# scylladb/seastar

Measured on AMD Instinct MI355X. Metric: GiB/s device-resident Internet checksum, 1500B-packet batches, 1/2/4/8 GPUs, higher is better.
Workload: dtype u8

## Files before the change

seastar_amd/csrc/sccsum.hip:

```cpp

#include <hip/hip_runtime.h>
#include "engine_seal.h"

#include <atomic>
#include <cctype>
#include <chrono>
#include <cstring>
#include <new>
#include <cstdint>
#include <cstdio>
#include <mutex>
#include <vector>

#include "host_launch.h"
#include "sccsum.h"
#include "sccsum_diag.h"

namespace sccsum {
namespace {

constexpr int kWave = 64;
constexpr int kBlock = 256;
constexpr int kWavesPerBlock = kBlock / kWave;
constexpr int kBlocksPerCU = 8;
// ... 800 lines not shown
        grp = group_of(wglob);
        const uint64_t rest = ntiles > nwaves ? ntiles - nwaves : 0;
        tiles_g = rest > grp ? static_cast<uint32_t>((rest - grp + kGroups - 1) / kGroups) : 0u;
        waves_g = static_cast<uint32_t>(nwaves / kGroups);
    }
    __device__ uint64_t end() const { return ntiles; }
    __device__ Ref ref(uint64_t tt) const {
        const bool sub = tt >= Q.tsplit;
        const uint64_t w = sub ? Q.tsplit + ((tt - Q.tsplit) >> Q.sub_log2) : tt;
        Ref r;
        r.q = 0;
        while (r.q + 1 < Q.nq && w >= Q.tile0[r.q + 1]) ++r.q;
        r.base = (w - Q.tile0[r.q]) * B;
        const uint64_t left = Q.n[r.q] - r.base;
        r.cnt = left < B ? static_cast<uint32_t>(left) : B;
        if (sub) {
            const uint32_t s0 = static_cast<uint32_t>((tt - Q.tsplit) & ((1u << Q.sub_log2) - 1u)) * Q.bsub;
            const uint32_t c = s0 < r.cnt ? r.cnt - s0 : 0u;
            r.base += s0 < r.cnt ? s0 : 0u;
            r.cnt = c < Q.bsub ? c : Q.bsub;
        }
        return r;
    }
    __device__ const uint8_t* bytes(const Ref& r) const { return Q.bytes[r.q]; }
    __device__ uint64_t bytes_len(const Ref& r) const { return Q.bytes_len[r.q]; }
    __device__ const uint64_t* off(const Ref& r) const { return Q.off[r.q]; }
    __device__ const uint32_t* len(const Ref& r) const { return Q.len[r.q]; }
    __device__ const uint32_t* seed(const Ref& r) const { return Q.seed[r.q]; }
    __device__ uint16_t* out(const Ref& r) const { return Q.out[r.q]; }
    __device__ uint8_t* status(const Ref& r) const { return Q.status[r.q]; }
    __device__ uint32_t tile_packets(const Ref&) const { return B; }
    __device__ bool is_store(const Ref&) const { return false; }
    __device__ uint32_t fill_flags(const Ref&, uint32_t flags) const { return flags; }
    __device__ uint32_t store_mode(const Ref&) const { return 0u; }

    struct Claim {
        uint32_t raw;
        uint64_t prev;
    };
    __device__ Claim claim_issue(uint64_t prev) {
        Claim c{0u, prev};
        if (heads != nullptr && lane == 0)
            c.raw = __hip_atomic_fetch_add(heads + grp * kHeadStride, 1u, __ATOMIC_RELAXED, __HIP_MEMORY_SCOPE_AGENT);
        return c;
    }
    __device__ uint64_t claim_resolve(const Claim& c) {
        if (heads == nullptr) return c.prev + nwaves;
        uint32_t d = c.raw;
        if (lane == 0 && d == tiles_g + waves_g - 1) {
            uint32_t* h = heads + grp * kHeadStride;
            __hip_atomic_store(h, 0u, __ATOMIC_RELAXED, __HIP_MEMORY_SCOPE_AGENT);
            asm volatile("s_waitcnt vmcnt(0)" ::: "memory");
            uint32_t* const groups_done = heads + kGroups * kHeadStride;
            const uint32_t gd = __hip_atomic_fetch_add(groups_done, 1u, __ATOMIC_RELAXED, __HIP_MEMORY_SCOPE_AGENT);
            if (gd == kGroups - 1) {
                __hip_atomic_store(groups_done, 0u, __ATOMIC_RELAXED, __HIP_MEMORY_SCOPE_AGENT);
                asm volatile("s_waitcnt vmcnt(0)" ::: "memory");
                __hip_atomic_store(done, ticket, __ATOMIC_RELAXED, __HIP_MEMORY_SCOPE_SYSTEM);
            }
        }
        d = __builtin_amdgcn_readfirstlane(d);
        return d < tiles_g ? nwaves + grp + static_cast<uint64_t>(kGroups) * d : ntiles;
    }
    __device__ uint64_t claim(uint64_t prev) { return claim_resolve(claim_issue(prev)); }
    __device__ uint64_t first() {
        uint64_t t = wglob;
        if (t >= ntiles && heads != nullptr) t = claim(t);
        return t;
    }
    __device__ bool ready(uint64_t) { return true; }
    __device__ bool wait_ready(uint64_t) { return true; }
    __device__ void retire(const Ref&) {}
};

constexpr uint32_t kEngineSlotWords = 64;
constexpr uint32_t kEngineCountSlots = 256;
constexpr uint32_t kEngineMaxRing = 1u << 16;
constexpr uint32_t kEngineDefaultRing = 1024;
#ifdef SCCSUM_AB_POLL_GROUP
constexpr uint32_t kPollGroup = SCCSUM_AB_POLL_GROUP;
#else
constexpr uint32_t kPollGroup = 16;
#endif
#ifdef SCCSUM_AB_NO_EXPECT
#define SCCSUM_HOT(x) (x)
#else
#define SCCSUM_HOT(x) __builtin_expect(!!(x), 1)
#endif
constexpr uint32_t kEdFirst = 0;
constexpr uint32_t kEdTiles = 1;
constexpr uint32_t kEdStep = 2;
constexpr uint32_t kEdNq = 3;
constexpr uint32_t kEdTile0 = 4;
constexpr uint32_t kEdQueue = 9;
constexpr uint32_t kEdKind = 41;
constexpr uint32_t kEdDep = 42;
constexpr uint32_t kEdIndex = 43;
constexpr uint32_t kStepSum = 0;
constexpr uint32_t kStepFillGen = 1;
constexpr uint32_t kStepFillStore = 2;
constexpr uint32_t kStoreTilePackets = 256;
constexpr uint32_t kEngineSyncEvery = 10;
#if defined(SCCSUM_AB_FILLSTORE_PLAIN) || defined(SCCSUM_AB_FILLSTORE_NORELEASE)
constexpr bool kStoreWT = false;
#else
constexpr bool kStoreWT = true;
#endif
constexpr uint32_t kEcPublished = 0, kEcStop = 8, kEcError = 16, kEcDone = 24;
constexpr uint64_t kErrIdle = 1, kErrDepWait = 2, kErrWalk = 3;
constexpr uint32_t kMpTiles = 0, kMpSteps = 8, kMpStop = 16, kMpToken = 24, kMpStamp = 32, kMirrorWords = 40;

struct EngineArgs {
    const uint64_t* hring;
    uint64_t* dring;
    uint64_t ring_mask;
    uint64_t* ctl;
    uint64_t* mirror;
    uint64_t* claims;
    uint32_t* counts;
    uint32_t* gdone;
    uint64_t* sdone;
    uint64_t idle_ticks;
    uint64_t dep_ticks;
};

__device__ __forceinline__ uint64_t rfl64(uint64_t x) {
    return static_cast<uint64_t>(static_cast<uint32_t>(__builtin_amdgcn_readfirstlane(static_cast<uint32_t>(x)))) |
           static_cast<uint64_t>(static_cast<uint32_t>(__builtin_amdgcn_readfirstlane(static_cast<uint32_t>(x >> 32))))
               << 32;
}
__device__ __forceinline__ uint64_t rl64(uint64_t x, uint32_t k) {
    return static_cast<uint64_t>(static_cast<uint32_t>(__builtin_amdgcn_readlane(static_cast<uint32_t>(x), k))) |
           static_cast<uint64_t>(static_cast<uint32_t>(__builtin_amdgcn_readlane(static_cast<uint32_t>(x >> 32), k)))
               << 32;
}

#ifdef SCCSUM_AB_NO_ENDPGM
__device__ __forceinline__ void engine_fault(uint64_t* ctl, uint32_t lane, uint64_t code) {
    if (lane == 0) __hip_atomic_store(ctl + kEcError, code, __ATOMIC_RELAXED, __HIP_MEMORY_SCOPE_SYSTEM);
}
#else
[[noreturn]] __device__ __forceinline__ void engine_fault(uint64_t* ctl, uint32_t lane, uint64_t code) {
    if (lane == 0) __hip_atomic_store(ctl + kEcError, code, __ATOMIC_RELAXED, __HIP_MEMORY_SCOPE_SYSTEM);
    asm volatile("s_waitcnt vmcnt(0)" ::: "memory");
    __builtin_amdgcn_endpgm();
}
#endif

struct WalkHit {
    uint64_t t, w;
};
__device__ __attribute__((noinline)) WalkHit engine_walk_far(const uint64_t* dring, uint64_t ring_mask,
                                                             const uint64_t* mirror, uint64_t* ctl, uint64_t below,
                                                             uint64_t v) {
    const uint32_t lane = __lane_id();
    uint64_t hs = 0;
    if (lane == 0) hs = __hip_atomic_load(mirror + kMpSteps, __ATOMIC_RELAXED, __HIP_MEMORY_SCOPE_AGENT);
    hs = rfl64(hs);
    uint64_t above = hs;
    bool bisect = false;
    uint64_t d = 1;
    for (;;) {
        uint64_t t;
        if (!bisect) {
            t = below + d;
            if (t >= above) {
                bisect = true;
                continue;
            }
        } else {
            if (above <= below + 1) break;
            t = below + (above - below) / 2;
        }
        uint64_t p = 0;
        if (lane == 0) p = __hip_atomic_load(dring + (t & ring_mask) * kEngineSlotWords + kEdStep, __ATOMIC_RELAXED,
                                             __HIP_MEMORY_SCOPE_AGENT);
        p = rfl64(p);
        if (seal_before(p, t, v)) {
            below = t;
            d <<= 1;
        } else {
            above = t;
            bisect = true;
        }
    }
    if (above >= hs) engine_fault(ctl, lane, kErrWalk);
    const uint64_t w = __hip_atomic_load(dring + (above & ring_mask) * kEngineSlotWords + lane, __ATOMIC_RELAXED,
                                         __HIP_MEMORY_SCOPE_AGENT);
    if (rl64(w, kEdIndex) != above || v < rl64(w, kEdFirst) || seal_before(rl64(w, kEdStep), above, v)) {
        engine_fault(ctl, lane, kErrWalk);
    }
    return WalkHit{above, w};
}

struct EngineSrc {
    static constexpr bool kEngine = true;
    const EngineArgs& E;
    const bool wt;
    uint32_t lane = 0, grp = 0;
    uint64_t pub = 0;
    uint64_t step = ~0ull, sfirst = 0, slast = 0;
    uint64_t dw = 0;
    uint64_t skind = 0, sdep = 0;
    uint64_t dep_seen = 0;
#ifdef SCCSUM_AB_TIMELINE
    unsigned long long ab[8] = {};
#endif
    struct Ref {
        uint32_t cnt, B, kind;
        uint64_t base, step, first, last;
        const uint8_t* bytes;
        uint64_t bytes_len;
        const uint64_t* off;
        const uint32_t* len;
        const uint32_t* seed;
        uint16_t* out;
        uint8_t* status;
    };
    __device__ EngineSrc(const EngineArgs& e, uint32_t flags) : E(e), wt((flags & kFlagEngineWT) != 0) {}
    __device__ void init(uint64_t wglob, uint64_t, uint32_t lane_) {
        lane = lane_;
        grp = group_of(wglob);
    }
    __device__ uint64_t end() const { return ~0ull; }
    struct Claim {
        uint64_t raw;
    };
    __device__ Claim claim_issue(uint64_t) {
        Claim c{0u};
        if (lane == 0) c.raw = __hip_atomic_fetch_add(E.claims + grp * (kHeadStride / 2), 1ull, __ATOMIC_RELAXED,
                                                      __HIP_MEMORY_SCOPE_AGENT);
        return c;
    }
    __device__ uint64_t claim_resolve(const Claim& c) {
        const uint64_t d = rfl64(c.raw);
        return grp + static_cast<uint64_t>(kGroups) * d;
    }
    __device__ uint64_t claim(uint64_t prev) { return claim_resolve(claim_issue(prev)); }
    __device__ uint64_t ctl_load(uint32_t w) {
        uint64_t v = 0;
        if (lane == 0) v = __hip_atomic_load(E.ctl + w, __ATOMIC_RELAXED, __HIP_MEMORY_SCOPE_SYSTEM);
        return rfl64(v);
    }
    __device__ uint64_t mload(uint32_t w) {
        uint64_t v = 0;
        if (lane == 0) v = __hip_atomic_load(E.mirror + w, __ATOMIC_RELAXED, __HIP_MEMORY_SCOPE_AGENT);
        return rfl64(v);
    }
    __device__ void poll() {
        uint32_t got = 0;
        if (lane == 0 && __hip_atomic_load(E.mirror + kMpToken, __ATOMIC_RELAXED, __HIP_MEMORY_SCOPE_AGENT) == 0) {
            uint64_t expect = 0;
            got = __hip_atomic_compare_exchange_strong(E.mirror + kMpToken, &expect, 1ull, __ATOMIC_RELAXED,
                                                       __ATOMIC_RELAXED, __HIP_MEMORY_SCOPE_AGENT)
                      ? 1u
                      : 0u;
        }
        if (!__builtin_amdgcn_readfirstlane(got)) return;
#ifdef SCCSUM_AB_TIMELINE
        ++ab[7];
#endif
        const uint64_t stop = ctl_load(kEcStop);
        const uint64_t hs = ctl_load(kEcPublished);
        uint64_t ms = mload(kMpSteps);
        const uint64_t ms0 = ms;
        uint64_t tiles = mload(kMpTiles);
        auto dslot = [&](uint64_t s) { return E.dring + (s & E.ring_mask) * kEngineSlotWords + lane; };
        auto put = [&](uint64_t s, uint64_t x) {
            __hip_atomic_store(dslot(s), x, __ATOMIC_RELAXED, __HIP_MEMORY_SCOPE_AGENT);
        };
        while (ms < hs) {
            const uint64_t g = hs - ms < kPollGroup ? hs - ms : kPollGroup;
            uint64_t w[kPollGroup];
#pragma unroll
            for (uint32_t k = 0; k < kPollGroup; ++k) {
                w[k] = k < g ? __hip_atomic_load(E.hring + ((ms + k) & E.ring_mask) * kEngineSlotWords + lane,
                                                 __ATOMIC_RELAXED, __HIP_MEMORY_SCOPE_SYSTEM)
                             : 0ull;
            }
#pragma unroll
            for (uint32_t k = 0; k < kPollGroup; ++k) {
                if (k < g) put(ms + k, w[k]);
            }
#pragma unroll
            for (uint32_t k = 0; k < kPollGroup; ++k) {
                if (k < g && static_cast<uint32_t>(rl64(w[k], kEdTiles)) == 0u && lane == 0) {
                    __hip_atomic_store(E.ctl + kEcDone + 8u * ((ms + k) & E.ring_mask), ms + k + 1, __ATOMIC_RELAXED,
                                       __HIP_MEMORY_SCOPE_SYSTEM);
                }
            }
#pragma unroll
            for (uint32_t k = 0; k < kPollGroup; ++k) {
                if (k + 1 == g) tiles = rl64(w[k], kEdFirst) + static_cast<uint32_t>(rl64(w[k], kEdTiles));
            }
            ms += g;
        }
        asm volatile("s_waitcnt vmcnt(0)" ::: "memory");
        if (lane == 0) __hip_atomic_store(E.mirror + kMpSteps, hs, __ATOMIC_RELAXED, __HIP_MEMORY_SCOPE_AGENT);
        asm volatile("s_waitcnt vmcnt(0)" ::: "memory");
        if (lane == 0) {
            __hip_atomic_store(E.mirror + kMpTiles, tiles, __ATOMIC_RELAXED, __HIP_MEMORY_SCOPE_AGENT);
            if (ms0 < hs) {
                __hip_atomic_store(E.mirror + kMpStamp, static_cast<uint64_t>(wall_clock64()), __ATOMIC_RELAXED,
                                   __HIP_MEMORY_SCOPE_AGENT);
            }
        }
        asm volatile("s_waitcnt vmcnt(0)" ::: "memory");
        if (lane == 0) {
            if (stop) __hip_atomic_store(E.mirror + kMpStop, 1ull, __ATOMIC_RELAXED, __HIP_MEMORY_SCOPE_AGENT);
            __hip_atomic_store(E.mirror + kMpToken, 0ull, __ATOMIC_RELAXED, __HIP_MEMORY_SCOPE_AGENT);
        }
    }
    __device__ bool published(uint64_t v) {
        if (SCCSUM_HOT(v < pub)) return true;
#ifdef SCCSUM_AB_TIMELINE
        ++ab[2];
#endif
        pub = mload(kMpTiles);
        return v < pub;
    }
    __device__ bool published_polled(uint64_t v) {
        if (published(v)) return true;
        poll();
        pub = mload(kMpTiles);
        return v < pub;
    }
    __device__ bool dep_ready(uint64_t v) {
        walk(v);
        if (SCCSUM_HOT(sdep == 0 || sdep <= dep_seen)) return true;
        const uint32_t slot = static_cast<uint32_t>((sdep - 1) % kEngineCountSlots);
        uint64_t d = 0;
        if (lane == 0) d = __hip_atomic_load(E.sdone + 8u * slot, __ATOMIC_RELAXED, __HIP_MEMORY_SCOPE_AGENT);
        d = rfl64(d);
        if (d < sdep) return false;
        dep_seen = sdep;
        return true;
    }
    __device__ bool ready(uint64_t v) { return published(v) && dep_ready(v); }
    __device__ bool wait_ready(uint64_t v) {
        if (ready(v)) return true;
        flush();
        const uint64_t t0 = static_cast<uint64_t>(wall_clock64());
#ifdef SCCSUM_AB_TIMELINE
        ++ab[0];
        struct Slept {
            unsigned long long* a;
            uint64_t t0;
            __device__ ~Slept() { a[1] += static_cast<uint64_t>(wall_clock64()) - t0; }
        } slept{ab, t0};
#endif
        for (;;) {
            const uint64_t stop = mload(kMpStop);
            const bool pubd = published_polled(v);
            if (pubd) {
                if (dep_ready(v)) return true;
                if (static_cast<uint64_t>(wall_clock64()) - t0 > E.dep_ticks) {
                    if (lane == 0) __hip_atomic_store(E.ctl + kEcError, kErrDepWait, __ATOMIC_RELAXED,
                                                      __HIP_MEMORY_SCOPE_SYSTEM);
                    return false;
                }
#ifdef SCCSUM_AB_DEP_SLEEP
                __builtin_amdgcn_s_sleep(SCCSUM_AB_DEP_SLEEP);
#else
                __builtin_amdgcn_s_sleep(32);
#endif
                continue;
            }
            if (stop) return false;
            const uint64_t now = static_cast<uint64_t>(wall_clock64());
            const uint64_t stamp = mload(kMpStamp);
            const uint64_t since = stamp > t0 ? stamp : t0;
            if (now > since && now - since > E.idle_ticks) {
                if (lane == 0) __hip_atomic_store(E.ctl + kEcError, kErrIdle, __ATOMIC_RELAXED,
                                                  __HIP_MEMORY_SCOPE_SYSTEM);
                return false;
            }
            __builtin_amdgcn_s_sleep(127);
        }
    }
    __device__ uint64_t first() {
        const uint64_t v = claim(0);
        return wait_ready(v) ? v : end();
    }
    __device__ void set_cursor(uint64_t t, uint64_t w) {
        step = t;
        dw = w;
        sfirst = rl64(w, kEdFirst);
        slast = sfirst + static_cast<uint32_t>(rl64(w, kEdTiles));
        skind = rl64(w, kEdKind);
        sdep = rl64(w, kEdDep);
    }
    __device__ bool walk(uint64_t v) {
        if (SCCSUM_HOT(step != ~0ull && v < slast)) return true;
#ifdef SCCSUM_AB_WALK_SEQ
        while (step == ~0ull || v >= slast) {
            const uint64_t t = step + 1;
            set_cursor(t, __hip_atomic_load(E.dring + (t & E.ring_mask) * kEngineSlotWords + lane, __ATOMIC_RELAXED,
                                            __HIP_MEMORY_SCOPE_AGENT));
        }
        return true;
#endif
#ifdef SCCSUM_AB_TIMELINE
        ++ab[3];
        const uint64_t w0 = static_cast<uint64_t>(wall_clock64());
        struct Walked {
            unsigned long long* a;
            uint64_t t0;
            __device__ ~Walked() { a[4] += static_cast<uint64_t>(wall_clock64()) - t0; }
        } walked{ab, w0};
#endif
        const uint64_t t = step + 1;
        const uint64_t w = __hip_atomic_load(E.dring + (t & E.ring_mask) * kEngineSlotWords + lane, __ATOMIC_RELAXED,
                                             __HIP_MEMORY_SCOPE_AGENT);
        if (SCCSUM_HOT(!seal_before(rl64(w, kEdStep), t, v) && rl64(w, kEdIndex) == t)) {
            set_cursor(t, w);
        } else {
            const WalkHit h = engine_walk_far(E.dring, E.ring_mask, E.mirror, E.ctl, t, v);
            set_cursor(rfl64(h.t), h.w);
        }
        return true;
    }
    __device__ Ref ref(uint64_t v) {
        Ref r;
        r.kind = static_cast<uint32_t>(skind);
        const uint64_t t_in = v - sfirst;
        const uint32_t nq = static_cast<uint32_t>(rl64(dw, kEdNq));
        uint32_t q = 0;
        while (q + 1 < nq && t_in >= rl64(dw, kEdTile0 + q + 1)) ++q;
        r.B = static_cast<uint32_t>(rl64(dw, kEdTiles) >> 32);
        r.base = (t_in - rl64(dw, kEdTile0 + q)) * r.B;
        const uint32_t qw = kEdQueue + 8u * q;
        const uint64_t left = rl64(dw, qw + 7) - r.base;
        r.cnt = left < r.B ? static_cast<uint32_t>(left) : r.B;
        r.bytes = reinterpret_cast<const uint8_t*>(rl64(dw, qw + 0));
        r.bytes_len = rl64(dw, qw + 1);
        r.off = reinterpret_cast<const uint64_t*>(rl64(dw, qw + 2));
        r.len = reinterpret_cast<const uint32_t*>(rl64(dw, qw + 3));
        r.seed = reinterpret_cast<const uint32_t*>(rl64(dw, qw + 4));
        r.out = reinterpret_cast<uint16_t*>(rl64(dw, qw + 5));
        r.status = reinterpret_cast<uint8_t*>(rl64(dw, qw + 6));
        r.step = step;
        r.first = sfirst;
        r.last = slast;
        return r;
    }
    __device__ const uint8_t* bytes(const Ref& r) const { return r.bytes; }
    __device__ uint64_t bytes_len(const Ref& r) const { return r.bytes_len; }
    __device__ const uint64_t* off(const Ref& r) const { return r.off; }
    __device__ const uint32_t* len(const Ref& r) const { return r.len; }
    __device__ const uint32_t* seed(const Ref& r) const { return r.seed; }
    __device__ uint16_t* out(const Ref& r) const { return r.out; }
    __device__ uint8_t* status(const Ref& r) const { return r.status; }
    __device__ uint32_t tile_packets(const Ref& r) const { return r.B; }
    __device__ bool is_store(const Ref& r) const { return (r.kind & 0xffu) == kStepFillStore; }
    __device__ uint32_t fill_flags(const Ref& r, uint32_t) const { return (r.kind >> 8) & 0xffu; }
    __device__ uint32_t store_mode(const Ref& r) const { return r.kind >> 16; }
    uint64_t pend_step = ~0ull, pend_first = 0, pend_last = 0;
    uint32_t pend = 0, pend_kind = 0;
#ifdef SCCSUM_AB_TIMELINE
    unsigned long long pend_t0 = 0, pend_t1 = 0;
#endif
    __device__ void flush() {
        if (pend == 0) return;
        const uint32_t k = pend;
        pend = 0;
#ifdef SCCSUM_AB_TIMELINE
        ++ab[5];
        struct Flushed {
            unsigned long long* a;
            uint64_t t0;
            __device__ ~Flushed() { a[6] += static_cast<uint64_t>(wall_clock64()) - t0; }
        } flushed{ab, static_cast<uint64_t>(wall_clock64())};
#endif
#ifdef SCCSUM_AB_TIMELINE
        if (lane == 0 && pend_step < kStepRec) {
            atomicMax(&g_step_grp[pend_step][grp], pend_t1);
            atomicMax(&g_step_xcd[pend_step][blockIdx.x & 7u][0], pend_t1);
            atomicMax(&g_step_xcd[pend_step][blockIdx.x & 7u][1], ~pend_t0);
        }
#endif
        if (lane != 0) return;
#ifdef SCCSUM_AB_FILLSTORE_NORELEASE
        if (false) {
#else
        if ((pend_kind & 0xffu) == kStepFillStore && !kStoreWT) {
#endif
            __builtin_amdgcn_fence(__ATOMIC_RELEASE, "");
        } else if (wt) {
            asm volatile("s_waitcnt vmcnt(0)" ::: "memory");
        } else {
            __builtin_amdgcn_fence(__ATOMIC_RELEASE, "agent");
        }
        const uint64_t fg = pend_first + ((grp + kGroups - pend_first % kGroups) % kGroups);
        const uint32_t expect = fg < pend_last ? static_cast<uint32_t>((pend_last - 1 - fg) / kGroups + 1) : 0u;
        const uint32_t slot = static_cast<uint32_t>(pend_step % kEngineCountSlots);
        uint32_t* const c = E.counts + (slot * kGroups + grp) * kHeadStride;
        const uint32_t x = __hip_atomic_fetch_add(c, k, __ATOMIC_RELAXED, __HIP_MEMORY_SCOPE_AGENT);
        if (x + k != expect) return;
        __hip_atomic_store(c, 0u, __ATOMIC_RELAXED, __HIP_MEMORY_SCOPE_AGENT);
        asm volatile("s_waitcnt vmcnt(0)" ::: "memory");
        uint32_t* const gd = E.gdone + slot * kHeadStride;
        const uint64_t ntl = pend_last - pend_first;
        const uint32_t groups = ntl < kGroups ? static_cast<uint32_t>(ntl) : kGroups;
        const uint32_t y = __hip_atomic_fetch_add(gd, 1u, __ATOMIC_RELAXED, __HIP_MEMORY_SCOPE_AGENT);
        if (y + 1 != groups) return;
        __hip_atomic_store(gd, 0u, __ATOMIC_RELAXED, __HIP_MEMORY_SCOPE_AGENT);
        __hip_atomic_store(E.sdone + 8u * slot, pend_step + 1, __ATOMIC_RELAXED, __HIP_MEMORY_SCOPE_AGENT);
        asm volatile("s_waitcnt vmcnt(0)" ::: "memory");
        __hip_atomic_store(E.ctl + kEcDone + 8u * (pend_step & E.ring_mask), pend_step + 1, __ATOMIC_RELAXED,
                           __HIP_MEMORY_SCOPE_SYSTEM);
    }
#ifdef SCCSUM_AB_TIMELINE
    __device__ void ab_stats(uint64_t wglob) {
        if (lane == 0 && wglob < kTimelineWaves)
            for (int i = 0; i < 8; ++i) g_engine_stats[wglob][i] = ab[i];
    }
#endif
    __device__ void retire(const Ref& r) {
        if (r.step != pend_step) {
            flush();
            pend_step = r.step;
            pend_first = r.first;
            pend_last = r.last;
            pend_kind = r.kind;
#ifdef SCCSUM_AB_TIMELINE
            pend_t0 = static_cast<uint64_t>(wall_clock64());
#endif
        }
        ++pend;
#ifdef SCCSUM_AB_TIMELINE
        pend_t1 = static_cast<uint64_t>(wall_clock64());
#endif
    }
};

template <bool kCoherent>
__device__ __forceinline__ uint32_t fill_ld32(const uint32_t* q) {
    if constexpr (kCoherent) {
        return __hip_atomic_load(gld(q), __ATOMIC_RELAXED, __HIP_MEMORY_SCOPE_AGENT);
    } else {
        return *gld(q);
    }
}
struct FillHead {
    uint32_t w, d0, d1, d2, d3;
};
template <bool kCoherent>
__device__ __forceinline__ FillHead fill_load(const uint8_t* p, const uint32_t* wp) {
    const uintptr_t a = reinterpret_cast<uintptr_t>(p);
    const uint32_t* d = reinterpret_cast<const uint32_t*>(a & ~uintptr_t(3));
    FillHead h;
    h.w = fill_ld32<kCoherent>(wp);
    h.d0 = fill_ld32<kCoherent>(d);
    h.d1 = fill_ld32<kCoherent>(d + 1);
    h.d2 = fill_ld32<kCoherent>(d + 2);
    h.d3 = fill_ld32<kCoherent>(d + 3);
    return h;
}
template <bool kCoherent, bool kWriteThrough = false>
__device__ __forceinline__ void fill_apply(uint8_t* p, uint32_t L, const FillHead& h, uint32_t mode) {
    const uint32_t sh = static_cast<uint32_t>(reinterpret_cast<uintptr_t>(p) & 3u);
    const uint32_t w = h.w, d0 = h.d0, d1 = h.d1, d2 = h.d2, d3 = h.d3;
    auto hbyte = [&](uint32_t k) {
        const uint32_t b = sh + k;
        const uint32_t dw = b < 4u ? d0 : (b < 8u ? d1 : (b < 12u ? d2 : d3));
        return (dw >> (8u * (b & 3u))) & 0xffu;
    };
    const uint32_t ihl = hbyte(0) & 0xfu;
    const uint32_t ip_len = (hbyte(2) << 8) | hbyte(3);
    const uint32_t fragw = (hbyte(6) << 8) | hbyte(7);
    const uint32_t proto = hbyte(9);
    const uint32_t l4_off = 4u * ihl;
    const uint32_t l4_end = ip_len < L ? ip_len : L;
    const bool atomic = !(L < ip_len || l4_off > l4_end || (fragw & 0x1fffu) * 8u + l4_end > 65535u ||
                          (fragw & 0x3fffu) != 0u || ihl < 5u);
    const uint32_t l4_len = l4_off > l4_end ? 0u : l4_end - l4_off;
    if (mode & SCCSUM_FILL_IP) store_field<kWriteThrough>(p + 10, w);
    if (!atomic) return;
    if (mode & SCCSUM_FILL_L4) {
        const uint32_t fo = proto == 17u ? 6u : (proto == 6u ? 16u : 0u);
        if (fo != 0u && l4_len >= fo + 2u) store_field<kWriteThrough>(p + l4_off + fo, w >> 16);
    }
    if ((mode & SCCSUM_FILL_ICMP_ECHO) && proto == 1u && l4_len >= 8u) {
        uint8_t* ih = p + l4_off;
        const uintptr_t ia = reinterpret_cast<uintptr_t>(ih);
        const uint32_t type = (fill_ld32<kCoherent>(reinterpret_cast<const uint32_t*>(ia & ~uintptr_t(3))) >>
                               (8u * static_cast<uint32_t>(ia & 3u))) & 0xffu;
        if (type == 8u) {
            store_field<kWriteThrough>(ih, 0u);
// ... 1505 lines not shown
    }
}

bool engine_all_done(sccsum_engine* e) {
    const uint64_t n = e->next_step.load(std::memory_order_relaxed);
    while (e->done_floor < n && engine_done(e, e->done_floor)) ++e->done_floor;
    return e->done_floor >= n;
}

int engine_check(const sccsum_engine* e, const sccsum_batch* batches, uint32_t nbatch, bool fill) {
    if (nbatch == 0 || nbatch > SCCSUM_ENGINE_MAX_BATCHES || !batches) return SCCSUM_EINVAL;
    for (uint32_t i = 0; i < nbatch; ++i) {
        const sccsum_batch& x = batches[i];
        if (e->frames && x.d_seed) return SCCSUM_EINVAL;
        if (!x.n) continue;
        const bool ok = e->frames
                            ? sccsum::batch_ok<true>(x.d_bytes, x.d_off, x.d_len, nullptr, x.d_out, x.d_status, 0)
                            : sccsum::batch_ok<false>(x.d_bytes, x.d_off, x.d_len, x.d_seed, x.d_out, x.d_status, 0);
        if (!ok) return SCCSUM_EINVAL;
        if (fill && !x.d_out) return SCCSUM_EINVAL;
    }
    return SCCSUM_OK;
}

bool engine_room(sccsum_engine* e, uint32_t k, uint64_t* need) {
    const uint64_t last = e->next_step.load(std::memory_order_relaxed) + k - 1;
    if (last < e->limit) return true;
    const uint64_t target = last - e->limit;
    while (e->done_floor <= target && engine_done(e, e->done_floor)) ++e->done_floor;
    if (e->done_floor > target) return true;
    *need = e->done_floor;
    return false;
}

uint64_t engine_tile(const sccsum_engine* e, const sccsum_batch* batches, uint32_t nbatch, uint32_t max_len) {
    uint64_t n_total = 0, bytes_total = 0;
    for (uint32_t i = 0; i < nbatch; ++i) {
        n_total += batches[i].n;
        bytes_total += batches[i].n ? batches[i].bytes_len : 0;
    }
    return sccsum::packets_per_tile(n_total, sccsum::packet_bytes(n_total, bytes_total, max_len), e->waves,
                                    sccsum::t_knobs);
}

uint64_t engine_put(sccsum_engine* e, const sccsum_batch* batches, uint32_t nbatch, uint64_t kind, uint64_t dep,
                    uint64_t B) {
    if ((kind & 0xffu) == sccsum::kStepFillStore) B = sccsum::kStoreTilePackets;
    const uint64_t s = e->next_step.load(std::memory_order_relaxed);
    uint64_t* const d = e->ring_h + (s & (e->ring - 1u)) * sccsum::kEngineSlotWords;
    uint64_t tile0[SCCSUM_ENGINE_MAX_BATCHES + 1] = {};
    uint32_t nq = 0;
    for (uint32_t i = 0; i < nbatch; ++i) {
        const sccsum_batch& x = batches[i];
        if (!x.n) continue;
        const uint32_t q = nq++;
        uint64_t* w = d + sccsum::kEdQueue + 8u * q;
        w[0] = reinterpret_cast<uint64_t>(x.d_bytes);
        w[1] = x.bytes_len;
        w[2] = reinterpret_cast<uint64_t>(x.d_off);
        w[3] = reinterpret_cast<uint64_t>(x.d_len);
        w[4] = e->frames ? 0u : reinterpret_cast<uint64_t>(x.d_seed);
        w[5] = reinterpret_cast<uint64_t>(x.d_out);
        w[6] = reinterpret_cast<uint64_t>(x.d_status);
        w[7] = x.n;
        tile0[q + 1] = tile0[q] + (x.n + B - 1) / B;
    }
    const uint64_t ntiles = tile0[nq];
    d[sccsum::kEdFirst] = e->next_first;
    d[sccsum::kEdTiles] = ntiles | (B << 32);
    d[sccsum::kEdStep] = sccsum::engine_seal(s, e->next_first + ntiles);
    d[sccsum::kEdIndex] = s;
    d[sccsum::kEdNq] = nq ? nq : 1;
    for (uint32_t q = 0; q <= SCCSUM_ENGINE_MAX_BATCHES; ++q) d[sccsum::kEdTile0 + q] = tile0[q];
    d[sccsum::kEdKind] = kind;
    d[sccsum::kEdDep] = dep;
    int sync = sccsum::t_knobs.engine_sync_every;
    if (sync < 0) sync = ntiles >= 2 * e->waves ? static_cast<int>(sccsum::kEngineSyncEvery) : 0;
    if (dep == 0 && sync > 0 && s > 0 && s % static_cast<uint64_t>(sync) == 0 && e->last_tiled != ~0ull) {
        d[sccsum::kEdDep] = e->last_tiled + 1;
    }
    if (ntiles) e->last_tiled = s;
    e->next_first += ntiles;
    e->next_step.store(s + 1, std::memory_order_release);
    __atomic_store_n(e->ctl_h + sccsum::kEcPublished, s + 1, __ATOMIC_SEQ_CST);
    return s;
}

template <class Put>
int engine_publish(sccsum_engine* e, uint32_t k, uint64_t timeout_ns, const Put& put) {
    const uint64_t t0 = now_ns();
    ProducerRecord* pr = nullptr;
    if (e->producer_limit) {
        uint64_t run;
        {
            std::lock_guard<std::mutex> g(e->mu);
            if (!e->running) return SCCSUM_EINVAL;
            run = e->run;
        }
        pr = &producer_record(e, run);
        while (pr->n >= e->producer_limit) {
            const uint64_t oldest = pr->steps[pr->head];
            const uint64_t spent = now_ns() - t0;
            const int rc = engine_wait_done(e, oldest, spent < timeout_ns ? timeout_ns - spent : 0);
            if (rc != SCCSUM_OK) return rc;
            pr->head = (pr->head + 1) % sccsum::kEngineCountSlots;
            --pr->n;
        }
    }
    for (;;) {
        uint64_t need = 0;
        {
            std::lock_guard<std::mutex> g(e->mu);
            if (!e->running) return SCCSUM_EINVAL;
            if (const int rc = engine_error(e)) return rc;
            if (engine_room(e, k, &need)) {
                put();
                if (pr) {
                    pr->steps[(pr->head + pr->n) % sccsum::kEngineCountSlots] =
                        e->next_step.load(std::memory_order_relaxed) - 1;
                    ++pr->n;
                }
                return SCCSUM_OK;
            }
        }
        const uint64_t spent = now_ns() - t0;
        const int rc = engine_wait_done(e, need, spent < timeout_ns ? timeout_ns - spent : 0);
        if (rc != SCCSUM_OK) return rc;
    }
}

int engine_ms(uint32_t ms, uint32_t dflt, uint64_t* ticks) {
    const uint64_t v = ms ? ms : dflt;
    if (v > 3600000u) return SCCSUM_EINVAL;
    *ticks = v * 100000ull;
    return SCCSUM_OK;
}

}

extern "C" {

int sccsum_engine_create_opts(int device, int mode, const sccsum_engine_opts* opts, sccsum_engine** out) {
    const int base = mode & ~SCCSUM_ENGINE_FILL;
    const bool fill = (mode & SCCSUM_ENGINE_FILL) != 0;
    if (!out || !opts || (base != SCCSUM_PIPE_IPV4 && base != SCCSUM_PIPE_SPANS) || (fill && base != SCCSUM_PIPE_IPV4)) {
        return SCCSUM_EINVAL;
    }
    const uint32_t ring_req = opts->ring_slots ? opts->ring_slots : sccsum::kEngineDefaultRing;
    const uint32_t mif = opts->max_in_flight ? opts->max_in_flight : 8u;
    uint64_t idle_ticks = 0, dep_ticks = 0;
    if (ring_req > sccsum::kEngineMaxRing || mif > sccsum::kEngineCountSlots || (fill && mif < 2) ||
        opts->producer_in_flight > mif ||
        engine_ms(opts->idle_ms, 1000u, &idle_ticks) != SCCSUM_OK || engine_ms(opts->dep_ms, 2000u, &dep_ticks) != SCCSUM_OK) {
        return SCCSUM_EINVAL;
    }
    uint32_t ring = 2;
    while (ring < ring_req) ring <<= 1;
    *out = nullptr;
    int n = 0;
    hipError_t e0 = hipGetDeviceCount(&n);
    if (e0 != hipSuccess) return static_cast<int>(e0);
    if (device < 0 || device >= n || device >= sccsum::kMaxDevices) return SCCSUM_ENODEV;
    const CurrentDevice keep;
    if ((e0 = hipSetDevice(device)) != hipSuccess) return static_cast<int>(e0);
    auto* e = new (std::nothrow) sccsum_engine;
    if (!e) return static_cast<int>(hipErrorOutOfMemory);
    e->device = device;
// ... 68 lines not shown
        if (w != hipSuccess) {
            release_live(e);
            return static_cast<int>(w);
        }
    }
    if (__atomic_load_n(e->ctl_h + sccsum::kEcError, __ATOMIC_ACQUIRE)) e->dirty = true;
    const uint64_t used = e->next_step.load(std::memory_order_relaxed);
    std::memset(e->ctl_h, 0, (sccsum::kEcDone + 8u * (used < e->ring ? used : e->ring)) * 8u);
    std::atomic_thread_fence(std::memory_order_seq_cst);
    hipError_t r = hipMemsetAsync(e->blk, 0, e->dirty ? EngineBlock::kBytes : EngineBlock::kReset, s);
    if (r != hipSuccess) {
        release_live(e);
        return static_cast<int>(r);
    }
    const sccsum::Knobs& K = sccsum::t_knobs;
    const uint32_t flags = sccsum::knob_flags(K) | (K.engine_wt ? sccsum::kFlagEngineWT : 0u);
    e->args.idle_ticks = K.engine_idle_ms > 0 ? static_cast<uint64_t>(K.engine_idle_ms) * 100000ull : e->idle_ticks;
    r = e->fill ? sccsum::launch_engine<true, true>(s, dev, e->args, flags, &e->waves)
                : (e->frames ? sccsum::launch_engine<true>(s, dev, e->args, flags, &e->waves)
                             : sccsum::launch_engine<false>(s, dev, e->args, flags, &e->waves));
    if (r != hipSuccess) {
        release_live(e);
        return static_cast<int>(r);
    }
    e->left_recorded = hipEventRecord(e->left, s) == hipSuccess;
    e->launched = true;
    e->stream = s;
    e->running = true;
    e->next_step.store(0, std::memory_order_release);
    e->next_first = 0;
    e->last_tiled = ~0ull;
    e->done_floor = 0;
    e->run = g_engine_runs.fetch_add(1, std::memory_order_relaxed) + 1;
    e->dirty = false;
    return SCCSUM_OK;
}

int sccsum_engine_submit(sccsum_engine* e, const sccsum_batch* batches, uint32_t nbatch, uint32_t max_len,
                         uint64_t timeout_ns, uint64_t* step) {
    if (!e || !step) return SCCSUM_EINVAL;
    if (const int rc = engine_check(e, batches, nbatch, false); rc != SCCSUM_OK) return rc;
    return engine_publish(e, 1, timeout_ns, [&] {
        *step = engine_put(e, batches, nbatch, sccsum::kStepSum, 0, engine_tile(e, batches, nbatch, max_len));
    });
}

int sccsum_engine_submit_fill(sccsum_engine* e, const sccsum_batch* batches, uint32_t nbatch, uint32_t max_len,
                              uint32_t mode, uint64_t timeout_ns, uint64_t* step) {
    constexpr uint32_t kEngineModes = SCCSUM_FILL_IP | SCCSUM_FILL_L4 | SCCSUM_FILL_ICMP_ECHO;
    if (!e || !step || !e->fill || (mode & ~kEngineModes) || !(mode & (SCCSUM_FILL_L4 | SCCSUM_FILL_ICMP_ECHO))) {
        return SCCSUM_EINVAL;
    }
    if (const int rc = engine_check(e, batches, nbatch, true); rc != SCCSUM_OK) return rc;
    uint64_t n_total = 0;
    for (uint32_t i = 0; i < nbatch; ++i) n_total += batches[i].n;
    const bool single = n_total <= sccsum::t_knobs.fill_single_max;
    const uint64_t kflags = sccsum::fill_flags(mode) | (single ? sccsum::kFlagFillNow : 0u);
    const uint64_t gen_kind = sccsum::kStepFillGen | (kflags << 8) | (uint64_t(mode) << 16);
    if (single) {
        return engine_publish(e, 1, timeout_ns, [&] {
            *step = engine_put(e, batches, nbatch, gen_kind, 0, engine_tile(e, batches, nbatch, max_len));
        });
    }
    sccsum_batch st[SCCSUM_ENGINE_MAX_BATCHES];
    for (uint32_t i = 0; i < nbatch; ++i) {
        st[i] = batches[i];
        st[i].d_status = nullptr;
    }
    return engine_publish(e, 2, timeout_ns, [&] {
        const uint64_t gen = engine_put(e, batches, nbatch, gen_kind, 0, engine_tile(e, batches, nbatch, max_len));
        *step = engine_put(e, st, nbatch, sccsum::kStepFillStore | (uint64_t(mode) << 16), gen + 1, 0);
    });
}

int sccsum_engine_wait(sccsum_engine* e, uint64_t step, uint64_t timeout_ns) {
    if (!e || step >= e->next_step.load(std::memory_order_acquire)) return SCCSUM_EINVAL;
    return engine_wait_done(e, step, timeout_ns);
}

int sccsum_engine_stop(sccsum_engine* e) {
    if (!e) return SCCSUM_EINVAL;
    std::lock_guard<std::mutex> g(e->mu);
    if (!e->running) return SCCSUM_EINVAL;
    __atomic_store_n(e->ctl_h + sccsum::kEcStop, 1ull, __ATOMIC_SEQ_CST);
    e->running = false;
    release_live(e);
    const int err = engine_error(e);
    return err && !engine_all_done(e) ? err : SCCSUM_OK;
}

int sccsum_engine_destroy(sccsum_engine* e) {
    if (!e) return SCCSUM_OK;
    bool running;
    {
        std::lock_guard<std::mutex> g(e->mu);
        running = e->running;
    }
    if (running) (void)sccsum_engine_stop(e);
    int rc = e->stream ? static_cast<int>(hipStreamSynchronize(e->stream)) : SCCSUM_OK;
    if (rc == SCCSUM_OK && e->launched) {
        std::lock_guard<std::mutex> g(e->mu);
        if (!engine_all_done(e)) rc = engine_error(e) ? engine_error(e) : SCCSUM_EFAULT;
    }
    (void)hipHostFree(e->ring_h);
    (void)hipHostFree(e->ctl_h);
    (void)hipFree(e->blk);
    (void)hipFree(e->args.dring);
    if (e->left) (void)hipEventDestroy(e->left);
    delete e;
    return rc;
}

int sccsum_abi_version(void) { return SCCSUM_ABI_VERSION; }

const char* sccsum_strerror(int err) {
    if (err == SCCSUM_OK) return "success";
    if (err == SCCSUM_EINVAL) return "invalid argument";
    if (err == SCCSUM_ENODEV) return "no such HIP device";
    if (err == SCCSUM_EBUSY) return "busy: every batch slot or engine step is in flight, or the device's engine is running";
    if (err == SCCSUM_EIDLE) return "the engine's grid gave up waiting for steps";
    if (err == SCCSUM_EFAULT) return "the engine's grid stopped on an internal fault";
    if (err > 0) return hipGetErrorString(static_cast<hipError_t>(err));
    return "unknown sccsum error";
}

int sccsum_device_count(int* count) {
    if (!count) return SCCSUM_EINVAL;
    return static_cast<int>(hipGetDeviceCount(count));
}

int sccsum_device_numa_node(int device, int* node) {
    if (!node) return SCCSUM_EINVAL;
    int n = 0;
    const hipError_t e = hipGetDeviceCount(&n);
    if (e != hipSuccess) return static_cast<int>(e);
    if (device < 0 || device >= n) return SCCSUM_ENODEV;
    char bdf[64] = {};
    const hipError_t e2 = hipDeviceGetPCIBusId(bdf, static_cast<int>(sizeof(bdf)), device);
    if (e2 != hipSuccess) return static_cast<int>(e2);
    for (char* c = bdf; *c; ++c) *c = static_cast<char>(std::tolower(static_cast<unsigned char>(*c)));
    char path[160];
    std::snprintf(path, sizeof(path), "/sys/bus/pci/devices/%s/numa_node", bdf);
    *node = -1;
    if (FILE* f = std::fopen(path, "r")) {
        int v = -1;
        if (std::fscanf(f, "%d", &v) == 1) *node = v;
        std::fclose(f);
    }
    return SCCSUM_OK;
}

int sccsum_init(int device) {
    int n = 0;
    const hipError_t e = hipGetDeviceCount(&n);
    if (e != hipSuccess) return static_cast<int>(e);
    if (device < 0 || device >= n) return SCCSUM_ENODEV;
    const hipError_t e2 = hipSetDevice(device);
    if (e2 != hipSuccess) return static_cast<int>(e2);
    (void)sccsum::cu_count(device);
    return sccsum::ensure_heads(device);
}

uint32_t sccsum_pseudo_seed(uint32_t src_host, uint32_t dst_host, uint8_t proto, uint16_t len) {
    uint64_t s = static_cast<uint64_t>(src_host) + dst_host + proto + len;
    while (s >> 16) s = (s & 0xffffu) + (s >> 16);
    return static_cast<uint32_t>(s);
}
// ... 286 lines not shown
```

Before: 6575.

## Pack stop flag into published words and streamline engine wait/poll paths

Folds the stop flag into the high bit of the published-step and mirror-tiles words, so each wait iteration does fewer control loads. Waiters near the front of the queue now sleep for a shorter interval, and the idle-timestamp load only happens once the idle timeout could have expired. Step lookup can search down from the newest published step when the target is nearer the head. Single-tile or single-group steps skip their counter atomics on completion. These changes add protocol complexity, and the host fetch_or on the published word can race with the publish store.

```diff
diff --git a/seastar_amd/csrc/sccsum.hip b/seastar_amd/csrc/sccsum.hip
--- a/seastar_amd/csrc/sccsum.hip
+++ b/seastar_amd/csrc/sccsum.hip
@@ -906,6 +906,11 @@
 #else
 constexpr uint32_t kPollGroup = 16;
 #endif
+#ifdef SCCSUM_AB_FRONT_SLEEP
+constexpr int kFrontSleep = SCCSUM_AB_FRONT_SLEEP;
+#else
+constexpr int kFrontSleep = 32;
+#endif
 #ifdef SCCSUM_AB_NO_EXPECT
 #define SCCSUM_HOT(x) (x)
 #else
@@ -930,9 +935,10 @@
 #else
 constexpr bool kStoreWT = true;
 #endif
-constexpr uint32_t kEcPublished = 0, kEcStop = 8, kEcError = 16, kEcDone = 24;
+constexpr uint32_t kEcPublished = 0, kEcError = 16, kEcDone = 24;
+constexpr uint64_t kStopBit = 1ull << 63;
 constexpr uint64_t kErrIdle = 1, kErrDepWait = 2, kErrWalk = 3;
-constexpr uint32_t kMpTiles = 0, kMpSteps = 8, kMpStop = 16, kMpToken = 24, kMpStamp = 32, kMirrorWords = 40;
+constexpr uint32_t kMpTiles = 0, kMpSteps = 8, kMpToken = 24, kMpStamp = 32, kMirrorWords = 40;
 
 struct EngineArgs {
     const uint64_t* hring;
@@ -976,24 +982,31 @@
 };
 __device__ __attribute__((noinline)) WalkHit engine_walk_far(const uint64_t* dring, uint64_t ring_mask,
                                                              const uint64_t* mirror, uint64_t* ctl, uint64_t below,
-                                                             uint64_t v) {
+                                                             uint64_t v, bool down) {
     const uint32_t lane = __lane_id();
     uint64_t hs = 0;
     if (lane == 0) hs = __hip_atomic_load(mirror + kMpSteps, __ATOMIC_RELAXED, __HIP_MEMORY_SCOPE_AGENT);
     hs = rfl64(hs);
     uint64_t above = hs;
+    if (down && hs > below + 1) {
+        const uint64_t t = hs - 1;
+        const uint64_t w = __hip_atomic_load(dring + (t & ring_mask) * kEngineSlotWords + lane, __ATOMIC_RELAXED,
+                                             __HIP_MEMORY_SCOPE_AGENT);
+        if (rl64(w, kEdIndex) == t && !seal_before(rl64(w, kEdStep), t, v)) {
+            if (rl64(w, kEdFirst) <= v) return WalkHit{t, w};
+            above = t;
+        } else {
+            below = t;
+        }
+    }
     bool bisect = false;
     uint64_t d = 1;
-    for (;;) {
+    while (above > below + 1) {
         uint64_t t;
-        if (!bisect) {
-            t = below + d;
-            if (t >= above) {
-                bisect = true;
-                continue;
-            }
+        if (!bisect && above - below > d) {
+            t = down ? above - d : below + d;
         } else {
-            if (above <= below + 1) break;
+            bisect = true;
             t = below + (above - below) / 2;
         }
         uint64_t p = 0;
@@ -1002,10 +1015,10 @@
         p = rfl64(p);
         if (seal_before(p, t, v)) {
             below = t;
-            d <<= 1;
+            if (down) bisect = true; else d <<= 1;
         } else {
             above = t;
-            bisect = true;
+            if (down) d <<= 1; else bisect = true;
         }
     }
     if (above >= hs) engine_fault(ctl, lane, kErrWalk);
@@ -1061,34 +1074,36 @@
         return grp + static_cast<uint64_t>(kGroups) * d;
     }
     __device__ uint64_t claim(uint64_t prev) { return claim_resolve(claim_issue(prev)); }
-    __device__ uint64_t ctl_load(uint32_t w) {
-        uint64_t v = 0;
-        if (lane == 0) v = __hip_atomic_load(E.ctl + w, __ATOMIC_RELAXED, __HIP_MEMORY_SCOPE_SYSTEM);
-        return rfl64(v);
-    }
     __device__ uint64_t mload(uint32_t w) {
         uint64_t v = 0;
         if (lane == 0) v = __hip_atomic_load(E.mirror + w, __ATOMIC_RELAXED, __HIP_MEMORY_SCOPE_AGENT);
         return rfl64(v);
     }
-    __device__ void poll() {
+    __device__ bool poll(bool token_free) {
         uint32_t got = 0;
-        if (lane == 0 && __hip_atomic_load(E.mirror + kMpToken, __ATOMIC_RELAXED, __HIP_MEMORY_SCOPE_AGENT) == 0) {
+        if (lane == 0 && token_free) {
             uint64_t expect = 0;
             got = __hip_atomic_compare_exchange_strong(E.mirror + kMpToken, &expect, 1ull, __ATOMIC_RELAXED,
                                                        __ATOMIC_RELAXED, __HIP_MEMORY_SCOPE_AGENT)
                       ? 1u
                       : 0u;
         }
-        if (!__builtin_amdgcn_readfirstlane(got)) return;
+        if (!__builtin_amdgcn_readfirstlane(got)) return false;
 #ifdef SCCSUM_AB_TIMELINE
         ++ab[7];
 #endif
-        const uint64_t stop = ctl_load(kEcStop);
-        const uint64_t hs = ctl_load(kEcPublished);
-        uint64_t ms = mload(kMpSteps);
+        uint64_t hw = 0, ms = 0, tiles = 0;
+        if (lane == 0) {
+            hw = __hip_atomic_load(E.ctl + kEcPublished, __ATOMIC_RELAXED, __HIP_MEMORY_SCOPE_SYSTEM);
+            ms = __hip_atomic_load(E.mirror + kMpSteps, __ATOMIC_RELAXED, __HIP_MEMORY_SCOPE_AGENT);
+            tiles = __hip_atomic_load(E.mirror + kMpTiles, __ATOMIC_RELAXED, __HIP_MEMORY_SCOPE_AGENT);
+        }
+        hw = rfl64(hw);
+        ms = rfl64(ms);
+        tiles = rfl64(tiles) & ~kStopBit;
+        const uint64_t stop = hw & kStopBit;
+        const uint64_t hs = hw & ~kStopBit;
         const uint64_t ms0 = ms;
-        uint64_t tiles = mload(kMpTiles);
         auto dslot = [&](uint64_t s) { return E.dring + (s & E.ring_mask) * kEngineSlotWords + lane; };
         auto put = [&](uint64_t s, uint64_t x) {
             __hip_atomic_store(dslot(s), x, __ATOMIC_RELAXED, __HIP_MEMORY_SCOPE_AGENT);
@@ -1123,30 +1138,22 @@
         if (lane == 0) __hip_atomic_store(E.mirror + kMpSteps, hs, __ATOMIC_RELAXED, __HIP_MEMORY_SCOPE_AGENT);
         asm volatile("s_waitcnt vmcnt(0)" ::: "memory");
         if (lane == 0) {
-            __hip_atomic_store(E.mirror + kMpTiles, tiles, __ATOMIC_RELAXED, __HIP_MEMORY_SCOPE_AGENT);
+            __hip_atomic_store(E.mirror + kMpTiles, tiles | stop, __ATOMIC_RELAXED, __HIP_MEMORY_SCOPE_AGENT);
             if (ms0 < hs) {
                 __hip_atomic_store(E.mirror + kMpStamp, static_cast<uint64_t>(wall_clock64()), __ATOMIC_RELAXED,
                                    __HIP_MEMORY_SCOPE_AGENT);
             }
         }
         asm volatile("s_waitcnt vmcnt(0)" ::: "memory");
-        if (lane == 0) {
-            if (stop) __hip_atomic_store(E.mirror + kMpStop, 1ull, __ATOMIC_RELAXED, __HIP_MEMORY_SCOPE_AGENT);
-            __hip_atomic_store(E.mirror + kMpToken, 0ull, __ATOMIC_RELAXED, __HIP_MEMORY_SCOPE_AGENT);
-        }
+        if (lane == 0) __hip_atomic_store(E.mirror + kMpToken, 0ull, __ATOMIC_RELAXED, __HIP_MEMORY_SCOPE_AGENT);
+        return true;
     }
     __device__ bool published(uint64_t v) {
         if (SCCSUM_HOT(v < pub)) return true;
 #ifdef SCCSUM_AB_TIMELINE
         ++ab[2];
 #endif
-        pub = mload(kMpTiles);
-        return v < pub;
-    }
-    __device__ bool published_polled(uint64_t v) {
-        if (published(v)) return true;
-        poll();
-        pub = mload(kMpTiles);
+        pub = mload(kMpTiles) & ~kStopBit;
         return v < pub;
     }
     __device__ bool dep_ready(uint64_t v) {
@@ -1165,6 +1172,7 @@
         if (ready(v)) return true;
         flush();
         const uint64_t t0 = static_cast<uint64_t>(wall_clock64());
+        uint64_t tdep = ~0ull;
 #ifdef SCCSUM_AB_TIMELINE
         ++ab[0];
         struct Slept {
@@ -1174,11 +1182,23 @@
         } slept{ab, t0};
 #endif
         for (;;) {
-            const uint64_t stop = mload(kMpStop);
-            const bool pubd = published_polled(v);
-            if (pubd) {
+            uint64_t stop = 0;
+            if (v >= pub) {
+                uint64_t m = 0, tok = 1;
+                if (lane == 0) {
+                    m = __hip_atomic_load(E.mirror + kMpTiles, __ATOMIC_RELAXED, __HIP_MEMORY_SCOPE_AGENT);
+                    tok = __hip_atomic_load(E.mirror + kMpToken, __ATOMIC_RELAXED, __HIP_MEMORY_SCOPE_AGENT);
+                }
+                m = rfl64(m);
+                if (v >= (m & ~kStopBit) && poll(tok == 0)) m = mload(kMpTiles);
+                pub = m & ~kStopBit;
+                stop = m & kStopBit;
+            }
+            if (v < pub) {
                 if (dep_ready(v)) return true;
-                if (static_cast<uint64_t>(wall_clock64()) - t0 > E.dep_ticks) {
+                const uint64_t now = static_cast<uint64_t>(wall_clock64());
+                if (tdep == ~0ull) tdep = now;
+                if (now - tdep > E.dep_ticks) {
                     if (lane == 0) __hip_atomic_store(E.ctl + kEcError, kErrDepWait, __ATOMIC_RELAXED,
                                                       __HIP_MEMORY_SCOPE_SYSTEM);
                     return false;
@@ -1192,14 +1212,20 @@
             }
             if (stop) return false;
             const uint64_t now = static_cast<uint64_t>(wall_clock64());
-            const uint64_t stamp = mload(kMpStamp);
-            const uint64_t since = stamp > t0 ? stamp : t0;
-            if (now > since && now - since > E.idle_ticks) {
-                if (lane == 0) __hip_atomic_store(E.ctl + kEcError, kErrIdle, __ATOMIC_RELAXED,
-                                                  __HIP_MEMORY_SCOPE_SYSTEM);
-                return false;
-            }
-            __builtin_amdgcn_s_sleep(127);
+            if (now - t0 > E.idle_ticks) {
+                const uint64_t stamp = mload(kMpStamp);
+                const uint64_t since = stamp > t0 ? stamp : t0;
+                if (now > since && now - since > E.idle_ticks) {
+                    if (lane == 0) __hip_atomic_store(E.ctl + kEcError, kErrIdle, __ATOMIC_RELAXED,
+                                                      __HIP_MEMORY_SCOPE_SYSTEM);
+                    return false;
+                }
+            }
+            if (v < pub + kGroups) {
+                __builtin_amdgcn_s_sleep(kFrontSleep);
+            } else {
+                __builtin_amdgcn_s_sleep(127);
+            }
         }
     }
     __device__ uint64_t first() {
@@ -1239,7 +1265,7 @@
         if (SCCSUM_HOT(!seal_before(rl64(w, kEdStep), t, v) && rl64(w, kEdIndex) == t)) {
             set_cursor(t, w);
         } else {
-            const WalkHit h = engine_walk_far(E.dring, E.ring_mask, E.mirror, E.ctl, t, v);
+            const WalkHit h = engine_walk_far(E.dring, E.ring_mask, E.mirror, E.ctl, t, v, pub - v < v - slast);
             set_cursor(rfl64(h.t), h.w);
         }
         return true;
@@ -1318,17 +1344,21 @@
         const uint64_t fg = pend_first + ((grp + kGroups - pend_first % kGroups) % kGroups);
         const uint32_t expect = fg < pend_last ? static_cast<uint32_t>((pend_last - 1 - fg) / kGroups + 1) : 0u;
         const uint32_t slot = static_cast<uint32_t>(pend_step % kEngineCountSlots);
-        uint32_t* const c = E.counts + (slot * kGroups + grp) * kHeadStride;
-        const uint32_t x = __hip_atomic_fetch_add(c, k, __ATOMIC_RELAXED, __HIP_MEMORY_SCOPE_AGENT);
-        if (x + k != expect) return;
-        __hip_atomic_store(c, 0u, __ATOMIC_RELAXED, __HIP_MEMORY_SCOPE_AGENT);
-        asm volatile("s_waitcnt vmcnt(0)" ::: "memory");
-        uint32_t* const gd = E.gdone + slot * kHeadStride;
+        if (expect != 1u) {
+            uint32_t* const c = E.counts + (slot * kGroups + grp) * kHeadStride;
+            const uint32_t x = __hip_atomic_fetch_add(c, k, __ATOMIC_RELAXED, __HIP_MEMORY_SCOPE_AGENT);
+            if (x + k != expect) return;
+            __hip_atomic_store(c, 0u, __ATOMIC_RELAXED, __HIP_MEMORY_SCOPE_AGENT);
+            asm volatile("s_waitcnt vmcnt(0)" ::: "memory");
+        }
         const uint64_t ntl = pend_last - pend_first;
-        const uint32_t groups = ntl < kGroups ? static_cast<uint32_t>(ntl) : kGroups;
-        const uint32_t y = __hip_atomic_fetch_add(gd, 1u, __ATOMIC_RELAXED, __HIP_MEMORY_SCOPE_AGENT);
-        if (y + 1 != groups) return;
-        __hip_atomic_store(gd, 0u, __ATOMIC_RELAXED, __HIP_MEMORY_SCOPE_AGENT);
+        if (ntl != 1u) {
+            uint32_t* const gd = E.gdone + slot * kHeadStride;
+            const uint32_t groups = ntl < kGroups ? static_cast<uint32_t>(ntl) : kGroups;
+            const uint32_t y = __hip_atomic_fetch_add(gd, 1u, __ATOMIC_RELAXED, __HIP_MEMORY_SCOPE_AGENT);
+            if (y + 1 != groups) return;
+            __hip_atomic_store(gd, 0u, __ATOMIC_RELAXED, __HIP_MEMORY_SCOPE_AGENT);
+        }
         __hip_atomic_store(E.sdone + 8u * slot, pend_step + 1, __ATOMIC_RELAXED, __HIP_MEMORY_SCOPE_AGENT);
         asm volatile("s_waitcnt vmcnt(0)" ::: "memory");
         __hip_atomic_store(E.ctl + kEcDone + 8u * (pend_step & E.ring_mask), pend_step + 1, __ATOMIC_RELAXED,
@@ -3000,7 +3030,8 @@
     if (ntiles) e->last_tiled = s;
     e->next_first += ntiles;
     e->next_step.store(s + 1, std::memory_order_release);
-    __atomic_store_n(e->ctl_h + sccsum::kEcPublished, s + 1, __ATOMIC_SEQ_CST);
+    const uint64_t stop = __atomic_load_n(e->ctl_h + sccsum::kEcPublished, __ATOMIC_RELAXED) & sccsum::kStopBit;
+    __atomic_store_n(e->ctl_h + sccsum::kEcPublished, (s + 1) | stop, __ATOMIC_SEQ_CST);
     return s;
 }
 
@@ -3235,7 +3266,7 @@
     if (!e) return SCCSUM_EINVAL;
     std::lock_guard<std::mutex> g(e->mu);
     if (!e->running) return SCCSUM_EINVAL;
-    __atomic_store_n(e->ctl_h + sccsum::kEcStop, 1ull, __ATOMIC_SEQ_CST);
+    __atomic_fetch_or(e->ctl_h + sccsum::kEcPublished, sccsum::kStopBit, __ATOMIC_SEQ_CST);
     e->running = false;
     release_live(e);
     const int err = engine_error(e);
```

Result: no change. 6576 (median of 2 runs) (+0.0%).
